# torognes/vsearch

Measured on AMD Instinct MI355X. Metric: GCUPS (useful DP cells/s of the search16 global-alignment path: DP + traceback + CIGAR), higher is better.
Workload: dtype int16

## Files before the change

### vsearch_amd/csrc/vsx_device.hip

```cpp
#include <hip/hip_runtime.h>
#include <type_traits>
#include <cstdlib>
#include <atomic>
#include "vsx_internal.h"

typedef unsigned int u32;
typedef unsigned int u32x4 __attribute__((ext_vector_type(4)));
typedef unsigned int u32x3 __attribute__((ext_vector_type(3)));
typedef short s2 __attribute__((ext_vector_type(2)));
typedef unsigned short us2 __attribute__((ext_vector_type(2)));

#define DEV __device__ __forceinline__
struct __attribute__((aligned(4))) Pair2 { unsigned int x, y; };

#define SIGN2 0x80008000u

DEV s2 S2(u32 x) { return __builtin_bit_cast(s2, x); }
DEV us2 U2(u32 x) { return __builtin_bit_cast(us2, x); }
DEV u32 UI(s2 x) { return __builtin_bit_cast(u32, x); }
DEV u32 UI(us2 x) { return __builtin_bit_cast(u32, x); }

DEV u32 sadd(u32 a, u32 b) { return UI(__builtin_elementwise_add_sat(S2(a), S2(b))); }
DEV u32 ssub(u32 a, u32 b) { return UI(__builtin_elementwise_sub_sat(S2(a), S2(b))); }
DEV u32 pmax(u32 a, u32 b) { return UI(__builtin_elementwise_max(S2(a), S2(b))); }
// ... 814 lines not shown
  static DEV u32 max(u32 a, u32 b) { return (u32) __builtin_elementwise_max((unsigned short) a, (unsigned short) b); }
  static DEV u32 dif(u32 a, u32 b) { return a - b; }
  static DEV u32 neg(u32 d) { return d >> 31; }
  static DEV u32 fun(u32 acc, u32 d) { return __builtin_amdgcn_alignbit(acc, d, 31); }
  static DEV u32 one_row_word(u32 acc) { return acc << 12; }
  static DEV u32 nibble(u32 w, int rows_in_group, int y) { return (w >> (4 * (rows_in_group - 1 - y))) & 15u; }
  static constexpr u32 UP = 8, LEFT = 4, EXT_UP = 2, EXT_LEFT = 1;
};

typedef u32 u32_unaligned __attribute__((aligned(1)));
typedef unsigned long long u64_unaligned __attribute__((aligned(1)));
struct __attribute__((aligned(4))) Quad { u32 x, y, z, w; };
struct __attribute__((aligned(4))) Trio { u32 x, y, z; };

#include "vsx_accept.h"

#ifndef VSX_TB_STATS
#define VSX_TB_STATS 0
#endif
#if VSX_TB_STATS
__device__ unsigned long long vsx_tb_stats_dev[16];
extern "C" hipError_t vsx_internal_tb_stats(unsigned long long * out8, int reset)
{
  hipError_t e = hipMemcpyFromSymbol(out8, HIP_SYMBOL(vsx_tb_stats_dev), sizeof(unsigned long long) * 16);
  if (e == hipSuccess && reset) { unsigned long long z[16] = {0}; e = hipMemcpyToSymbol(HIP_SYMBOL(vsx_tb_stats_dev), z, sizeof z); }
  return e;
}
#endif

#ifndef VSX_TB_WAVES
#define VSX_TB_WAVES(R_, MID_) ((MID_) ? ((R_) <= 24 ? 4 : 3) : ((R_) <= 12 ? 4 : ((R_) <= 16 ? 3 : 2)))
#endif
template <int R, bool FAST, bool CK8 = false, bool MID = false>
__global__ void __launch_bounds__(128) __attribute__((amdgpu_waves_per_eu(VSX_TB_WAVES(R, MID), 8)))
vsx_traceback_ck_kernel(const VsxDevParams P, const VsxFilterDev FL, const VsxTask * __restrict__ tasks,
                        const u32 * __restrict__ pair_slot, const u32 * __restrict__ pair_ids, u32 npairs,
                        const uint8_t * __restrict__ qc, const uint8_t * __restrict__ tc,
                        const u32 * __restrict__ ck, const VsxSlotOut * __restrict__ slot,
                        u32 * __restrict__ slab, const uint64_t * __restrict__ slab_off,
                        u32 * __restrict__ runs, uint64_t runs_capacity, unsigned long long * cursor,
                        VsxPairOut * __restrict__ out)
{
  typedef TbOps<FAST> A;
  static_assert(VSX_RB == 1, "the tile staging below reads row checkpoints as two-step (16-byte) pairs");
  static_assert(!CK8 || FAST, "compressed checkpoints belong to the TILT class");
  static_assert(!MID || (CK8 && R % 2 == 0), "half-height tiles belong to the TILT class");
  constexpr int RT = MID ? R / 2 : R;
  constexpr int ND = (RT + 3) / 4;
  constexpr bool TOPPAD = FAST;
  typedef typename std::conditional<CK8, uint8_t, int16_t>::type SshT;
  __shared__ SshT Ssh[512];
  __shared__ uint16_t bitsL_all[2 * 16 * ND * 64];
  __shared__ u32 tbL_all[2 * 17 * 64];
  __shared__ uint8_t symL_all[2 * 8 * 64];
  const int tid = (int) (threadIdx.x & 63);
  const int wv = (int) (threadIdx.x >> 6);
// ... 375 lines not shown
              if (op == 1 && (bts & A::EXT_LEFT)) { --j; push(1); }
              else if (op == 2 && (bts & A::EXT_UP)) { --i; --r; push(2); }
              else if (bts & A::LEFT) { if (op != 1) ++ga; --j; push(1); }
              else if (bts & A::UP) { if (op != 2) ++ga; --i; --r; push(2); }
              else { --i; --r; --j; push(0); }
#if VSX_TB_STATS
              atomicAdd(&vsx_tb_stats_dev[3], 1ull);
#endif
            }
          if (r < 0 && L > 0) { --L; r = (L == 0 ? rtop0 : R) - 1; }
        }
    }
#if VSX_TB_STATS
  if (valid) atomicAdd(&vsx_tb_stats_dev[5], 1ull);
#endif
  if (!valid) return;

  VsxPairOut o;
  o.pad = 0; o.nruns = 0; o.run_off = 0;
  if (so.overflow)
    {
      o.score = 32767; o.aligned = 0; o.matches = 0; o.mismatches = 0; o.gaps = 0;
      out[pair_ids[k]] = o;
      rank_note(FL, pair_ids[k], 0u, 32767, 0.0);
      return;
    }
  if (i >= 0) { al += (u32) (i + 1); if (op != 2) ++ga; push_n(2, (u32) (i + 1)); }
  if (j >= 0) { al += (u32) (j + 1); if (op != 1) ++ga; push_n(1, (u32) (j + 1)); }
  if (op >= 0) my[nruns++] = (runlen << 2) | (u32) op;

  u32 ma = 0, mi = 0;
  {
    int qi = Q - 1, tj = D - 1;
    for (u32 x = 0; x < nruns; ++x)
      {
        const u32 w = my[x];
        const int len = (int) (w >> 2);
        const u32 o2 = w & 3u;
        if (o2 == 0)
          {
            for (int b = 0; b < len; b += 8)
              {
                const int rem = (len - b < 8) ? len - b : 8;
                const unsigned long long aw = *reinterpret_cast<const u64_unaligned *>(q + (qi - b - 7));
                const unsigned long long cw = *reinterpret_cast<const u64_unaligned *>(d + (tj - b - 7));
                const unsigned long long ones = 0x0101010101010101ull;
                const unsigned long long x = aw & cw;
                unsigned long long t = (x | (x >> 1) | (x >> 2) | (x >> 3)) & ones;
                if (P.n_mismatch)
                  {
                    const unsigned long long a15 = aw & (aw >> 1) & (aw >> 2) & (aw >> 3);
                    const unsigned long long c15 = cw & (cw >> 1) & (cw >> 2) & (cw >> 3);
                    t &= ~(a15 | c15);
                  }
                t &= ~0ull << (8 * (8 - rem));
                const u32 m8 = (u32) __builtin_popcountll(t);
                ma += m8;
                mi += (u32) rem - m8;
              }
            qi -= len; tj -= len;
          }
        else if (o2 == 1) tj -= len;
        else qi -= len;
      }
  }

  u32 verdict = 0;
  double idv = 0.0;
  if (FL.enabled && nruns > 0) verdict = accept_verdict(FL, Q, D, (int) al, (int) ma, (int) mi, (int) ga, my[nruns - 1], my[0], &idv);
  if (verdict == 3u) nruns = 0;
  rank_note(FL, pair_ids[k], verdict, (int) so.score, idv);

  const unsigned long long base = atomicAdd(cursor, (unsigned long long) nruns);
  if (base + nruns <= runs_capacity)
    for (u32 x = 0; x < nruns; ++x) runs[base + x] = my[x];

  o.score = so.score;
  o.aligned = (uint16_t) al; o.matches = (uint16_t) ma; o.mismatches = (uint16_t) mi; o.gaps = (uint16_t) ga;
  o.pad = (uint16_t) verdict;
  o.nruns = nruns;
  o.run_off = base;
  out[pair_ids[k]] = o;
}


DEV u32 pk_add(u32 a, u32 b) { return UI((us2) (U2(a) + U2(b))); }
DEV u32 pk_sub(u32 a, u32 b) { return psubw(a, b); }
#ifdef VSX_TB2_WAVES_N
#define VSX_TB2_WAVES(R_, MID_) VSX_TB2_WAVES_N
#endif
#ifndef VSX_TB2_WAVES
#define VSX_TB2_WAVES(R_, MID_) 3
#endif
#ifndef VSX_TB_LDSSTAGE
#define VSX_TB_LDSSTAGE 1
#endif
#ifndef VSX_TB_LDSSTAGE_FOR
#define VSX_TB_LDSSTAGE_FOR(R_) ((R_) == 14 || (R_) == 16 || (R_) >= 26)
#endif
#ifndef VSX_TB_WALK_BATCH
#define VSX_TB_WALK_BATCH 4
#endif
static_assert(VSX_TB_WALK_BATCH >= 1 && VSX_TB_WALK_BATCH <= 16, "a batch stays inside one 16-column tile");
template <int R, bool MID>
__global__ void __launch_bounds__(64) __attribute__((amdgpu_waves_per_eu(VSX_TB2_WAVES(R, MID), 8)))
vsx_traceback_tilt_kernel(const VsxDevParams P, const VsxFilterDev FL, const VsxTask * __restrict__ tasks,
                          const u32 * __restrict__ pair_slot, const u32 * __restrict__ pair_ids, u32 npairs,
                          const uint8_t * __restrict__ qc, const uint8_t * __restrict__ tc,
                          const u32 * __restrict__ ck, const VsxSlotOut * __restrict__ slot,
                          u32 * __restrict__ slab, const uint64_t * __restrict__ slab_off,
                          u32 * __restrict__ runs, uint64_t runs_capacity, unsigned long long * cursor,
                          VsxPairOut * __restrict__ out)
{
  static_assert(R >= 4 && (!MID || R % 2 == 0), "R = 1 keeps the first kernel");
  constexpr int RT = MID ? R / 2 : R;
  constexpr int HR = (RT + 1) / 2;
  constexpr int NG = (HR + 3) / 4;
  constexpr int XL = RT - 1 - HR;
  constexpr int WB = VSX_TB_WALK_BATCH;
  constexpr int NBQ = MID ? VSX_COLCK_NBH(RT) : VSX_COLCK_NB(R, true);
  __shared__ uint8_t Ssh[512];
  __shared__ u32 Ssh4[16];
  constexpr int BITS_DW = 17 * NG * 64, SYM_DW = 10 * 64 / 4;
  __shared__ __attribute__((aligned(16))) u32 arenaL[BITS_DW + SYM_DW + 19 * 64];
  u32 * const bitsL = arenaL;
  uint8_t * const symL = reinterpret_cast<uint8_t *>(arenaL + BITS_DW);
  u32 * const tbL = arenaL + BITS_DW + SYM_DW;
// ... 458 lines not shown
#endif
          TBMARK(3 * tno + 2);
        }
      if (busy && r < 0 && L > 0) { --L; r = R - 1; }
    }
#if VSX_TB_STATS
  if (valid) atomicAdd(&vsx_tb_stats_dev[5], 1ull);
  if (n_cells) atomicAdd(&vsx_tb_stats_dev[3], (unsigned long long) n_cells);
  if (tid == 0)
    {
      atomicAdd(&vsx_tb_stats_dev[15], __builtin_readcyclecounter() - t_kernel0); atomicAdd(&vsx_tb_stats_dev[0], (unsigned long long) n_iter);
      atomicAdd(&vsx_tb_stats_dev[4], (unsigned long long) n_trips);
      for (int k2 = 0; k2 < 6; ++k2) atomicAdd(&vsx_tb_stats_dev[8 + k2], tphase[k2]);
    }
#endif
  if (!valid) return;

  VsxPairOut o;
  o.pad = 0; o.nruns = 0; o.run_off = 0;
  if (so.overflow)
    {
      o.score = 32767; o.aligned = 0; o.matches = 0; o.mismatches = 0; o.gaps = 0;
      out[pair_ids[k]] = o;
      rank_note(FL, pair_ids[k], 0u, 32767, 0.0);
      return;
    }
  if (i >= 0) { al += (u32) (i + 1); if (op != 2) ++ga; push_n(2, (u32) (i + 1)); }
  if (j >= 0) { al += (u32) (j + 1); if (op != 1) ++ga; push_n(1, (u32) (j + 1)); }
  if (op >= 0) my[nruns++] = (runlen << 2) | (u32) op;

  u32 ma = 0, mi = 0;
  {
    int qi = Q - 1, tj = D - 1;
    for (u32 x = 0; x < nruns; ++x)
      {
        const u32 w = my[x];
        const int len = (int) (w >> 2);
        const u32 o2 = w & 3u;
        if (o2 == 0)
          {
            for (int b = 0; b < len; b += 8)
              {
                const int rem = (len - b < 8) ? len - b : 8;
                const unsigned long long aw = *reinterpret_cast<const u64_unaligned *>(q + (qi - b - 7));
                const unsigned long long cw = *reinterpret_cast<const u64_unaligned *>(d + (tj - b - 7));
                const unsigned long long ones = 0x0101010101010101ull;
                const unsigned long long x2 = aw & cw;
                unsigned long long t = (x2 | (x2 >> 1) | (x2 >> 2) | (x2 >> 3)) & ones;
                if (P.n_mismatch)
                  {
                    const unsigned long long a15 = aw & (aw >> 1) & (aw >> 2) & (aw >> 3);
                    const unsigned long long c15 = cw & (cw >> 1) & (cw >> 2) & (cw >> 3);
                    t &= ~(a15 | c15);
                  }
                t &= ~0ull << (8 * (8 - rem));
                const u32 m8 = (u32) __builtin_popcountll(t);
                ma += m8;
                mi += (u32) rem - m8;
              }
            qi -= len; tj -= len;
          }
        else if (o2 == 1) tj -= len;
        else qi -= len;
      }
  }

  u32 verdict = 0;
  double idv = 0.0;
  if (FL.enabled && nruns > 0) verdict = accept_verdict(FL, Q, D, (int) al, (int) ma, (int) mi, (int) ga, my[nruns - 1], my[0], &idv);
  if (verdict == 3u) nruns = 0;
  rank_note(FL, pair_ids[k], verdict, (int) so.score, idv);

  const unsigned long long base = atomicAdd(cursor, (unsigned long long) nruns);
  if (base + nruns <= runs_capacity)
    for (u32 x = 0; x < nruns; ++x) runs[base + x] = my[x];

  o.score = so.score;
  o.aligned = (uint16_t) al; o.matches = (uint16_t) ma; o.mismatches = (uint16_t) mi; o.gaps = (uint16_t) ga;
  o.pad = (uint16_t) verdict;
  o.nruns = nruns;
  o.run_off = base;
  out[pair_ids[k]] = o;
}

DEV u32 map4(u32 ch)
{
  const u32 c = ch | 0x20u;
  if (((ch | 0x20u) < 'a') || ((ch | 0x20u) > 'z') || ((ch & 0xC0u) != 0x40u)) return 0;
  switch (c)
    {
    case 'a': return 1;  case 'b': return 14; case 'c': return 2;  case 'd': return 13;
    case 'g': return 4;  case 'h': return 11; case 'k': return 12; case 'm': return 3;
    case 'n': return 15; case 'r': return 5;  case 's': return 6;  case 't': return 8;
    case 'u': return 8;  case 'v': return 7;  case 'w': return 9;  case 'y': return 10;
    default: return 0;
    }
}
// ... 169 lines not shown
{
  if (ntasks == 0) return hipSuccess;
#define FWDR(RR) case RR: return launch_fwd2<RR>(track, nq, one, P, d_tasks, ntasks, q, t, dir, strip, slot, st)
  switch (rows)
    {
    FWDR(1); FWDR(4); FWDR(8); FWDR(10); FWDR(12); FWDR(14); FWDR(16); FWDR(18); FWDR(20); FWDR(22); FWDR(24); FWDR(26); FWDR(28); FWDR(32);
    default: return hipErrorInvalidValue;
    }
#undef FWDR
}

template <int R, bool MID>
static hipError_t launch_tbtilt(const VsxDevParams & P, const VsxFilterDev & F, const VsxTask * d_tasks, const uint32_t * d_pair_slot,
                                const uint32_t * d_pair_ids, uint32_t npairs, const uint8_t * q, const uint8_t * t,
                                const uint32_t * ck, const VsxSlotOut * slot, uint32_t * slab, const uint64_t * slab_off,
                                uint32_t * runs, uint64_t cap, unsigned long long * cursor, VsxPairOut * out, hipStream_t st)
{
  if constexpr (R >= 4)
    hipLaunchKernelGGL((vsx_traceback_tilt_kernel<R, MID>), dim3((npairs + 63) / 64), dim3(64), 0, st,
                       P, F, d_tasks, d_pair_slot, d_pair_ids, npairs, q, t, ck, slot, slab, slab_off, runs, cap, cursor, out);
  return hipGetLastError();
}

template <int R, bool FAST, bool CK8 = false, bool MID = false>
static hipError_t launch_tbck(const VsxDevParams & P, const VsxFilterDev & F, const VsxTask * d_tasks, const uint32_t * d_pair_slot,
                              const uint32_t * d_pair_ids, uint32_t npairs, const uint8_t * q, const uint8_t * t,
                              const uint32_t * ck, const VsxSlotOut * slot, uint32_t * slab, const uint64_t * slab_off,
                              uint32_t * runs, uint64_t cap, unsigned long long * cursor, VsxPairOut * out, hipStream_t st)
{
  hipLaunchKernelGGL((vsx_traceback_ck_kernel<R, FAST, CK8, MID>), dim3((npairs + 127) / 128), dim3(128), 0, st,
                     P, F, d_tasks, d_pair_slot, d_pair_ids, npairs, q, t, ck, slot, slab, slab_off, runs, cap, cursor, out);
  return hipGetLastError();
}

extern "C" hipError_t vsx_launch_traceback_ck(int rows, int fast16, VsxDevParams P, VsxFilterDev F, const VsxTask * d_tasks, const uint32_t * d_pair_slot,
                                              const uint32_t * d_pair_ids, uint32_t npairs,
                                              const uint8_t * q, const uint8_t * t,
                                              const uint32_t * ck, const VsxSlotOut * slot,
                                              uint32_t * slab, const uint64_t * slab_off,
                                              uint32_t * runs, uint64_t runs_capacity, unsigned long long * cursor,
                                              VsxPairOut * out, hipStream_t st)
{
  if (npairs == 0) return hipSuccess;
  int dev_now = 0;
  if (hipGetDevice(&dev_now) != hipSuccess) { (void) hipGetLastError(); dev_now = 64; }
  const bool v2 = g_tb_v1_dev[dev_now < 0 || dev_now > 64 ? 64 : dev_now].load(std::memory_order_relaxed) == 0;
#define TBCK(RR) case RR: return (fast16 && P.tilt != 0 && v2 && RR >= 4) ? launch_tbtilt<RR, VSX_MID(RR, true)>(P, F, d_tasks, d_pair_slot, d_pair_ids, npairs, q, t, ck, slot, slab, slab_off, runs, runs_capacity, cursor, out, st) \
                                 : (fast16 && P.tilt != 0) ? launch_tbck<RR, true, true, VSX_MID(RR, true)>(P, F, d_tasks, d_pair_slot, d_pair_ids, npairs, q, t, ck, slot, slab, slab_off, runs, runs_capacity, cursor, out, st) \
                                 : fast16 ? launch_tbck<RR, true>(P, F, d_tasks, d_pair_slot, d_pair_ids, npairs, q, t, ck, slot, slab, slab_off, runs, runs_capacity, cursor, out, st) \
                                        : launch_tbck<RR, false>(P, F, d_tasks, d_pair_slot, d_pair_ids, npairs, q, t, ck, slot, slab, slab_off, runs, runs_capacity, cursor, out, st)
  switch (rows)
    {
    TBCK(1); TBCK(4); TBCK(8); TBCK(10); TBCK(12); TBCK(14); TBCK(16); TBCK(18); TBCK(20); TBCK(22); TBCK(24); TBCK(26); TBCK(28); TBCK(32);
    default: return hipErrorInvalidValue;
    }
#undef TBCK
}

extern "C" uint64_t vsx_ckpt_dwords(uint64_t nstrips, uint64_t steps, uint64_t rows, int tilt)
{
  const uint64_t nblk = (steps + 15) >> 4;
  const uint64_t rowck = (((nstrips * steps) + 1) >> 1) * VSX_ROWCK_PAIR_DW(tilt != 0);
  if (tilt)
    {
      const bool mid = VSX_MID(rows, true);
// ... 8 lines not shown
```

### vsearch_amd/csrc/vsx_host.cpp

```cpp
#include "../../include/vsx.h"
#include "vsx_internal.h"
#include "vsx_private.h"

#include <hip/hip_runtime.h>
#include <algorithm>
#include <cerrno>
#include <cinttypes>
#include <cstdio>
#include <cstdlib>
#include <cstring>
#include <sched.h>
#include <thread>
#include <atomic>
#include <condition_variable>
#include <mutex>
#include <chrono>
#include <deque>
#include <functional>
#include <memory>
#include <numeric>
#include <string>
#include <vector>

using vsxp::fail;
// ... 1456 lines not shown
  pl->filter.refused_pair = pl->d_refused_pair.p;
  return VSX_OK;
}

int vsx_plan_run(vsx_plan * pl)
{
  if (!pl) return fail(VSX_EINVAL, "vsx_plan_run: null plan");
  vsx_ctx * ctx = pl->ctx;
  VSX_HIP(hipSetDevice(ctx->device));
  hipStream_t st = pl->alt_fwd ? ctx->stream_b : ctx->stream, st2 = ctx->stream2;
  const int slot = pl->dir_slot;
  const int poison = vsx_internal_poison_byte();
  VSX_HIP(hipMemsetAsync(pl->d_cursor.p, 0, 3 * sizeof(unsigned long long), st));
  if (pl->filter.rank_counts) VSX_HIP(hipMemsetAsync(pl->d_rank_counts.p, 0, 2 * sizeof(uint32_t), st));
  VSX_HIP(hipEventRecord(pl->ev_begin, st));
  for (size_t k = 0; k < pl->chunks.size(); ++k)
    {
      Chunk & c = pl->chunks[k];
      uint32_t * dir = pl->d_dir[0].p;
      if (k >= 1) VSX_HIP(hipStreamWaitEvent(st, pl->chunks[k - 1].e2, 0));
      else if (ctx->ev_tb_used[slot]) VSX_HIP(hipStreamWaitEvent(st, ctx->ev_tb[slot], 0));
      if (poison >= 0)
        {
          VSX_HIP(hipMemsetAsync(dir, poison, (c.dir_dwords + VSX_CK_SLACK_DW) * sizeof(uint32_t), st));
          if (c.strip_elems) VSX_HIP(hipMemsetAsync(pl->d_strip.p, poison, c.strip_elems * sizeof(uint2), st));
        }
      VSX_HIP(hipEventRecord(c.e0, st));
      for (const Launch & L : c.launches)
        {
          VsxDevParams Pf = L.tilt ? ctx->Pt : ctx->P;
// ... 8 lines not shown
      VSX_HIP(hipStreamWaitEvent(st2, c.e1, 0));
      if (poison >= 0 && c.slab_words) VSX_HIP(hipMemsetAsync(pl->d_slab.p, poison, c.slab_words * sizeof(uint32_t), st2));
      VSX_HIP(hipEventRecord(c.e1b, st2));
      for (size_t li = 0; li < c.launches.size();)
        {
          const Launch & L = c.launches[li];
          uint32_t pair_count = L.pair_count;
          size_t lj = li + 1;
          while (lj < c.launches.size() && c.launches[lj].rows == L.rows &&
                 c.launches[lj].track == L.track && c.launches[lj].tilt == L.tilt) { pair_count += c.launches[lj].pair_count; ++lj; }
          VsxDevParams Pb = L.tilt ? ctx->Pt : ctx->P;
          Pb.max3 = (L.tilt == 2) ? 1 : 0;
          VSX_HIP(vsx_launch_traceback_ck(L.rows, L.track == 0 ? 1 : 0, Pb, pl->filter, pl->d_tasks.p, pl->d_pair_slot.p + L.pair_first,
                                         pl->d_pair_ids.p + L.pair_first, pair_count, pl->Q->codes(), pl->T->codes(),
                                         dir, pl->d_slot.p, pl->d_slab.p, pl->d_slab_off.p + L.pair_first,
                                         pl->d_runs.p, pl->runs_capacity, pl->d_cursor.p, pl->d_out.p, st2));
          li = lj;
        }
      VSX_HIP(hipEventRecord(c.e2, st2));
    }
  if (pl->chunks.empty()) VSX_HIP(hipStreamWaitEvent(st2, pl->ev_begin, 0));
  VSX_HIP(hipEventRecord(ctx->ev_tb[slot], st2));
  ctx->ev_tb_used[slot] = true;
  VSX_HIP(vsx_launch_cigar_text(pl->d_out.p, pl->d_pair_ids.p, (uint32_t) pl->pair_ids.size(), pl->d_runs.p, pl->runs_capacity,
                               pl->d_text.p, pl->text_capacity, pl->d_cursor.p + 1, pl->soa, st2));
  VSX_HIP(hipMemcpyAsync(pl->h_cursor, pl->d_cursor.p, 3 * sizeof(unsigned long long), hipMemcpyDeviceToHost, st2));
  VSX_HIP(hipEventRecord(pl->ev_end, st2));
  pl->ran = true;
  pl->host_patched = false;
  return VSX_OK;
}

int vsx_plan_sync(vsx_plan * pl, vsx_timing * tm)
{
  if (!pl) return fail(VSX_EINVAL, "vsx_plan_sync: null plan");
  if (!pl->ran) return fail(VSX_EINVAL, "vsx_plan_sync: plan has not been run");
  VSX_HIP(hipSetDevice(pl->ctx->device));
  VSX_HIP(hipEventSynchronize(pl->ev_end));
  if (tm)
    {
// ... 622 lines not shown
```

### vsearch_amd/csrc/vsx_internal.h

```cpp
#ifndef VSX_INTERNAL_H
#define VSX_INTERNAL_H

#include <stdint.h>
#include <hip/hip_runtime_api.h>

#define VSX_TASK_SLOTS 8
#define VSX_GROUP_LANES 16
#define VSX_MAX_SEQLEN_SUM 65535LL
#define VSX_MAX_SEQLEN_PRODUCT 25000000LL
#define VSX_TABLE_LEN (65536 + 64)
#define VSX_CODE_SLACK 64
#define VSX_CK_SLACK_DW 4096
#ifndef VSX_MID_MIN_ROWS
#define VSX_MID_MIN_ROWS 18
#endif
#define VSX_MID(R_, TILT_) ((TILT_) && (R_) >= VSX_MID_MIN_ROWS)
#define VSX_SPLIT_ROWS(R_) ((R_) == 10 || (R_) == 16)

struct VsxDevParams {
  uint32_t match_pk;
  uint32_t qrq_i_pk, rq_i_pk;
  uint32_t qrq_r_pk, rq_r_pk;
  int32_t  qrt_i, rt_i;
  int32_t  qrt_r, rt_r;
  int32_t  match, mismatch;
  int32_t  smin;
  int32_t  n_mismatch;
  int32_t  share_sub;
  int32_t  top_open, top_step;
  int32_t  tilt;
  int32_t  max3;
  int32_t  es_on, es_w0, es_e, es_rr, es_rate;
// ... 35 lines not shown
struct VsxPairOut {
  int16_t  score;
  uint16_t aligned, matches, mismatches, gaps;
  uint16_t pad;
  uint32_t nruns;
  uint64_t run_off;
};

struct VsxSoaOut {
  int16_t  * score;
  uint16_t * aligned, * matches, * mismatches, * gaps;
  uint8_t  * verdict;
  uint64_t * text_off;
};

struct VsxRankedOut {
  uint32_t * pair;
  int16_t  * score;
  uint16_t * aligned, * matches, * mismatches, * gaps;
  uint8_t  * verdict;
  double   * id;
  uint64_t * text_off;
};

#define VSX_CHIM_MAXCAND 16
struct VsxChimItem {
  uint32_t q;
  uint32_t ncand;
  uint32_t pair0;
  uint32_t out;
// ... 47 lines not shown
hipError_t vsx_launch_revcomp(uint8_t * d_codes, const uint64_t * d_src_off, const uint64_t * d_dst_off,
                              const uint32_t * d_len, uint64_t nseq, hipStream_t st);

hipError_t vsx_launch_encode(const uint8_t * d_ascii, uint8_t * d_codes, uint64_t nbytes, hipStream_t st);
hipError_t vsx_launch_purity(const uint8_t * d_codes, const uint64_t * d_off, const uint32_t * d_len,
                             uint64_t nseq, uint8_t * d_impure, hipStream_t st);
hipError_t vsx_launch_forward(int rows, int track, int nq, int one , VsxDevParams P, const VsxTask * d_tasks, uint32_t ntasks,
                              const uint8_t * d_qcodes, const uint8_t * d_tcodes,
                              uint32_t * d_dir, uint2 * d_strip, VsxSlotOut * d_slot, hipStream_t st);
hipError_t vsx_launch_traceback_ck(int rows, int fast16, VsxDevParams P, VsxFilterDev F, const VsxTask * d_tasks, const uint32_t * d_pair_slot,
                                   const uint32_t * d_pair_ids, uint32_t npairs,
                                   const uint8_t * d_qcodes, const uint8_t * d_tcodes,
                                   const uint32_t * d_ck, const VsxSlotOut * d_slot,
                                   uint32_t * d_slab, const uint64_t * d_slab_off,
                                   uint32_t * d_runs, uint64_t runs_capacity, unsigned long long * d_cursor,
                                   VsxPairOut * d_out, hipStream_t st);
hipError_t vsx_launch_max3_selftest(uint32_t * d_bad , hipStream_t st);
void vsx_internal_set_tb_v2(int device, int on);
uint64_t vsx_ckpt_dwords(uint64_t nstrips, uint64_t steps, uint64_t rows, int tilt );
const int * vsx_supported_rows(int * count);

hipError_t vsx_kmer_launch_sweep(int fill, const uint8_t * codes, const uint64_t * off, const uint32_t * len,
                                 const uint32_t * seq_list, uint32_t nseq, int w, uint32_t ntiles, uint32_t * bucket_count,
                                 const uint64_t * bucket_start, uint32_t * postings, const uint8_t * lower_bits, hipStream_t st);
hipError_t vsx_kmer_launch_case_bits(const uint8_t * d_ascii, uint64_t nbytes, uint8_t * d_bits , int fold_case,
                                     hipStream_t st);
hipError_t vsx_launch_dust(const uint8_t * d_codes, const uint64_t * d_off, const uint32_t * d_len, uint64_t nseq, uint8_t * d_bits,
                           hipStream_t st);
hipError_t vsx_kmer_launch_ranges(const uint64_t * bucket_start, uint32_t ntiles, const uint64_t * qk_start, const uint32_t * qk,
                                  const uint32_t * minmatch, const uint32_t * qlist, uint32_t nslots, void * ranges, hipStream_t st);
hipError_t vsx_kmer_launch_count(int bits, int tagged, const uint32_t * postings, const uint64_t * bucket_start, const void * ranges,
// ... 25 lines not shown
```

### vsearch_amd/csrc/vsx_tbtext.hip

```cpp
#include <hip/hip_runtime.h>
#include "vsx_internal.h"

typedef unsigned int u32;

#define DEV __device__ __forceinline__

DEV u32 ndigits(u32 v) { return v >= 10000u ? 5u : v >= 1000u ? 4u : v >= 100u ? 3u : v >= 10u ? 2u : 1u; }

__global__ void __launch_bounds__(256)
vsx_cigar_text_kernel(const VsxPairOut * __restrict__ out, const u32 * __restrict__ pair_ids, u32 npairs,
                      const u32 * __restrict__ runs, uint64_t runs_capacity,
                      uint8_t * __restrict__ text, uint64_t text_capacity, unsigned long long * text_cursor,
                      VsxSoaOut soa)
{
  const u32 k = blockIdx.x * blockDim.x + threadIdx.x;
  const bool valid = k < npairs;
  const u32 pid = valid ? pair_ids[k] : 0u;
  VsxPairOut o {};
  if (valid) o = out[pid];
  const bool have_runs = valid && (o.run_off + o.nruns <= runs_capacity);
  const u32 * __restrict__ my = runs + o.run_off;
  const u32 nruns = have_runs ? o.nruns : 0u;

  u32 len = 1;
  for (u32 x = 0; x < nruns; ++x)
    {
      const u32 n = my[x] >> 2;
      len += 1u + (n > 1u ? ndigits(n) : 0u);
    }
  const u32 len4 = valid ? ((len + 3u) & ~3u) : 0u;

  u32 incl = len4;
#pragma unroll
  for (int d = 1; d < 64; d <<= 1)
    {
      const u32 v = (u32) __shfl_up((int) incl, d, 64);
      if ((int) (threadIdx.x & 63) >= d) incl += v;
    }
  const u32 total = (u32) __shfl((int) incl, 63, 64);
  unsigned long long base = 0;
  if ((threadIdx.x & 63) == 0 && total) base = atomicAdd(text_cursor, (unsigned long long) total);
  base = (unsigned long long) __shfl((long long) base, 0, 64);
  if (!valid) return;
  const unsigned long long off = base + (unsigned long long) (incl - len4);

  if (off + len4 <= text_capacity)
    {
      u32 * __restrict__ dst = reinterpret_cast<u32 *>(text + off);
      u32 acc = 0, have = 0;
      auto put = [&](u32 ch) {
        acc |= ch << (8u * have);
        if (++have == 4u) { *dst++ = acc; acc = 0; have = 0; }
      };
      for (u32 x = nruns; x-- > 0;)
        {
          const u32 w = my[x];
          const u32 n = w >> 2;
          if (n > 1u)
            {
              if (n >= 10000u) put('0' + n / 10000u);
              if (n >= 1000u) put('0' + (n / 1000u) % 10u);
              if (n >= 100u) put('0' + (n / 100u) % 10u);
              if (n >= 10u) put('0' + (n / 10u) % 10u);
              put('0' + n % 10u);
            }
          put((w & 3u) == 0u ? 'M' : (w & 3u) == 1u ? 'I' : 'D');
        }
      put(0u);
      if (have) *dst = acc;
    }

  soa.score[pid] = o.score;
  soa.aligned[pid] = o.aligned;
  soa.matches[pid] = o.matches;
  soa.mismatches[pid] = o.mismatches;
  soa.gaps[pid] = o.gaps;
  soa.verdict[pid] = (uint8_t) o.pad;
  soa.text_off[pid] = off;
}

__global__ void __launch_bounds__(256)
vsx_revcomp_kernel(const uint8_t * __restrict__ codes, const uint64_t * __restrict__ src_off, const uint64_t * __restrict__ dst_off,
                   const uint32_t * __restrict__ len)
{
  const uint64_t k = blockIdx.x;
  const uint8_t * __restrict__ s = codes + src_off[k];
  uint8_t * __restrict__ d = const_cast<uint8_t *>(codes) + dst_off[k];
  const u32 L = len[k];
  for (u32 x = threadIdx.x; x < L; x += 256)
    {
      const u32 c = s[L - 1 - x] & 15u;
      const u32 r = ((c & 1u) << 3) | ((c & 2u) << 1) | ((c & 4u) >> 1) | ((c & 8u) >> 3);
      d[x] = (uint8_t) (c == 0u ? 15u : r);
// ... 22 lines not shown
```

Measured before the change: 9578.

## Fuse CIGAR text formatting into traceback kernels

The traceback kernels now format the CIGAR text and write the SoA outputs themselves, using a wave-wide prefix scan to allocate text space. This replaces the separate cigar-text kernel launch, so the run words no longer go to global memory and come back. The writer fills the string back to front so runs can be emitted in stored order. The trade is extra registers and work in the traceback kernels, and the early returns are restructured so every lane reaches the wave-wide shuffle.

```diff
diff --git a/vsearch_amd/csrc/vsx_device.hip b/vsearch_amd/csrc/vsx_device.hip
--- a/vsearch_amd/csrc/vsx_device.hip
+++ b/vsearch_amd/csrc/vsx_device.hip
@@ -852,6 +852,7 @@
 struct __attribute__((aligned(4))) Trio { u32 x, y, z; };
 
 #include "vsx_accept.h"
+#include "vsx_tbtext.h"
 
 #ifndef VSX_TB_STATS
 #define VSX_TB_STATS 0
@@ -877,7 +878,7 @@
                         const u32 * __restrict__ ck, const VsxSlotOut * __restrict__ slot,
                         u32 * __restrict__ slab, const uint64_t * __restrict__ slab_off,
                         u32 * __restrict__ runs, uint64_t runs_capacity, unsigned long long * cursor,
-                        VsxPairOut * __restrict__ out)
+                        VsxPairOut * __restrict__ out, const VsxTextOut TX)
 {
   typedef TbOps<FAST> A;
   static_assert(VSX_RB == 1, "the tile staging below reads row checkpoints as two-step (16-byte) pairs");
@@ -1283,73 +1284,83 @@
 #if VSX_TB_STATS
   if (valid) atomicAdd(&vsx_tb_stats_dev[5], 1ull);
 #endif
-  if (!valid) return;
-
+  const u32 pid = valid ? pair_ids[k] : 0u;
+  bool have_runs = true;
+  u32 tlen = 1;
   VsxPairOut o;
   o.pad = 0; o.nruns = 0; o.run_off = 0;
-  if (so.overflow)
-    {
-      o.score = 32767; o.aligned = 0; o.matches = 0; o.mismatches = 0; o.gaps = 0;
-      out[pair_ids[k]] = o;
-      rank_note(FL, pair_ids[k], 0u, 32767, 0.0);
-      return;
-    }
-  if (i >= 0) { al += (u32) (i + 1); if (op != 2) ++ga; push_n(2, (u32) (i + 1)); }
-  if (j >= 0) { al += (u32) (j + 1); if (op != 1) ++ga; push_n(1, (u32) (j + 1)); }
-  if (op >= 0) my[nruns++] = (runlen << 2) | (u32) op;
-
-  u32 ma = 0, mi = 0;
-  {
-    int qi = Q - 1, tj = D - 1;
-    for (u32 x = 0; x < nruns; ++x)
+  o.score = 32767; o.aligned = 0; o.matches = 0; o.mismatches = 0; o.gaps = 0;
+  if (valid && so.overflow)
+    {
+      out[pid] = o;
+      rank_note(FL, pid, 0u, 32767, 0.0);
+    }
+  if (live)
+    {
+      if (i >= 0) { al += (u32) (i + 1); if (op != 2) ++ga; push_n(2, (u32) (i + 1)); }
+      if (j >= 0) { al += (u32) (j + 1); if (op != 1) ++ga; push_n(1, (u32) (j + 1)); }
+      if (op >= 0) my[nruns++] = (runlen << 2) | (u32) op;
+
+      u32 ma = 0, mi = 0;
       {
-        const u32 w = my[x];
-        const int len = (int) (w >> 2);
-        const u32 o2 = w & 3u;
-        if (o2 == 0)
+        int qi = Q - 1, tj = D - 1;
+        for (u32 x = 0; x < nruns; ++x)
           {
-            for (int b = 0; b < len; b += 8)
+            const u32 w = my[x];
+            const int len = (int) (w >> 2);
+            if (VSX_TB_FUSED_TEXT) tlen += vsx_cigar_run_len(w);
+            const u32 o2 = w & 3u;
+            if (o2 == 0)
               {
-                const int rem = (len - b < 8) ? len - b : 8;
-                const unsigned long long aw = *reinterpret_cast<const u64_unaligned *>(q + (qi - b - 7));
-                const unsigned long long cw = *reinterpret_cast<const u64_unaligned *>(d + (tj - b - 7));
-                const unsigned long long ones = 0x0101010101010101ull;
-                const unsigned long long x = aw & cw;
-                unsigned long long t = (x | (x >> 1) | (x >> 2) | (x >> 3)) & ones;
-                if (P.n_mismatch)
+                for (int b = 0; b < len; b += 8)
                   {
-                    const unsigned long long a15 = aw & (aw >> 1) & (aw >> 2) & (aw >> 3);
-                    const unsigned long long c15 = cw & (cw >> 1) & (cw >> 2) & (cw >> 3);
-                    t &= ~(a15 | c15);
+                    const int rem = (len - b < 8) ? len - b : 8;
+                    const unsigned long long aw = *reinterpret_cast<const u64_unaligned *>(q + (qi - b - 7));
+                    const unsigned long long cw = *reinterpret_cast<const u64_unaligned *>(d + (tj - b - 7));
+                    const unsigned long long ones = 0x0101010101010101ull;
+                    const unsigned long long x = aw & cw;
+                    unsigned long long t = (x | (x >> 1) | (x >> 2) | (x >> 3)) & ones;
+                    if (P.n_mismatch)
+                      {
+                        const unsigned long long a15 = aw & (aw >> 1) & (aw >> 2) & (aw >> 3);
+                        const unsigned long long c15 = cw & (cw >> 1) & (cw >> 2) & (cw >> 3);
+                        t &= ~(a15 | c15);
+                      }
+                    t &= ~0ull << (8 * (8 - rem));
+                    const u32 m8 = (u32) __builtin_popcountll(t);
+                    ma += m8;
+                    mi += (u32) rem - m8;
                   }
-                t &= ~0ull << (8 * (8 - rem));
-                const u32 m8 = (u32) __builtin_popcountll(t);
-                ma += m8;
-                mi += (u32) rem - m8;
+                qi -= len; tj -= len;
               }
-            qi -= len; tj -= len;
+            else if (o2 == 1) tj -= len;
+            else qi -= len;
           }
-        else if (o2 == 1) tj -= len;
-        else qi -= len;
       }
-  }
-
-  u32 verdict = 0;
-  double idv = 0.0;
-  if (FL.enabled && nruns > 0) verdict = accept_verdict(FL, Q, D, (int) al, (int) ma, (int) mi, (int) ga, my[nruns - 1], my[0], &idv);
-  if (verdict == 3u) nruns = 0;
-  rank_note(FL, pair_ids[k], verdict, (int) so.score, idv);
-
-  const unsigned long long base = atomicAdd(cursor, (unsigned long long) nruns);
-  if (base + nruns <= runs_capacity)
-    for (u32 x = 0; x < nruns; ++x) runs[base + x] = my[x];
-
-  o.score = so.score;
-  o.aligned = (uint16_t) al; o.matches = (uint16_t) ma; o.mismatches = (uint16_t) mi; o.gaps = (uint16_t) ga;
-  o.pad = (uint16_t) verdict;
-  o.nruns = nruns;
-  o.run_off = base;
-  out[pair_ids[k]] = o;
+
+      u32 verdict = 0;
+      double idv = 0.0;
+      if (FL.enabled && nruns > 0) verdict = accept_verdict(FL, Q, D, (int) al, (int) ma, (int) mi, (int) ga, my[nruns - 1], my[0], &idv);
+      if (verdict == 3u) nruns = 0;
+      rank_note(FL, pid, verdict, (int) so.score, idv);
+
+      const unsigned long long base = atomicAdd(cursor, (unsigned long long) nruns);
+      have_runs = base + nruns <= runs_capacity;
+      if (!VSX_TB_FUSED_TEXT && have_runs)
+        for (u32 x = 0; x < nruns; ++x) runs[base + x] = my[x];
+
+      o.score = so.score;
+      o.aligned = (uint16_t) al; o.matches = (uint16_t) ma; o.mismatches = (uint16_t) mi; o.gaps = (uint16_t) ga;
+      o.pad = (uint16_t) verdict;
+      o.nruns = nruns;
+      o.run_off = base;
+      out[pid] = o;
+    }
+#if VSX_TB_FUSED_TEXT
+  vsx_marshal_pair(valid, pid, o, my, have_runs ? o.nruns : 0u, tlen, runs, TX);
+#else
+  (void) tlen;
+#endif
 }
 
 
@@ -1379,7 +1390,7 @@
                           const u32 * __restrict__ ck, const VsxSlotOut * __restrict__ slot,
                           u32 * __restrict__ slab, const uint64_t * __restrict__ slab_off,
                           u32 * __restrict__ runs, uint64_t runs_capacity, unsigned long long * cursor,
-                          VsxPairOut * __restrict__ out)
+                          VsxPairOut * __restrict__ out, const VsxTextOut TX)
 {
   static_assert(R >= 4 && (!MID || R % 2 == 0), "R = 1 keeps the first kernel");
   constexpr int RT = MID ? R / 2 : R;
@@ -1868,73 +1879,83 @@
       for (int k2 = 0; k2 < 6; ++k2) atomicAdd(&vsx_tb_stats_dev[8 + k2], tphase[k2]);
     }
 #endif
-  if (!valid) return;
-
+  const u32 pid = valid ? pair_ids[k] : 0u;
+  bool have_runs = true;
+  u32 tlen = 1;
   VsxPairOut o;
   o.pad = 0; o.nruns = 0; o.run_off = 0;
-  if (so.overflow)
-    {
-      o.score = 32767; o.aligned = 0; o.matches = 0; o.mismatches = 0; o.gaps = 0;
-      out[pair_ids[k]] = o;
-      rank_note(FL, pair_ids[k], 0u, 32767, 0.0);
-      return;
-    }
-  if (i >= 0) { al += (u32) (i + 1); if (op != 2) ++ga; push_n(2, (u32) (i + 1)); }
-  if (j >= 0) { al += (u32) (j + 1); if (op != 1) ++ga; push_n(1, (u32) (j + 1)); }
-  if (op >= 0) my[nruns++] = (runlen << 2) | (u32) op;
-
-  u32 ma = 0, mi = 0;
-  {
-    int qi = Q - 1, tj = D - 1;
-    for (u32 x = 0; x < nruns; ++x)
+  o.score = 32767; o.aligned = 0; o.matches = 0; o.mismatches = 0; o.gaps = 0;
+  if (valid && so.overflow)
+    {
+      out[pid] = o;
+      rank_note(FL, pid, 0u, 32767, 0.0);
+    }
+  if (live)
+    {
+      if (i >= 0) { al += (u32) (i + 1); if (op != 2) ++ga; push_n(2, (u32) (i + 1)); }
+      if (j >= 0) { al += (u32) (j + 1); if (op != 1) ++ga; push_n(1, (u32) (j + 1)); }
+      if (op >= 0) my[nruns++] = (runlen << 2) | (u32) op;
+
+      u32 ma = 0, mi = 0;
       {
-        const u32 w = my[x];
-        const int len = (int) (w >> 2);
-        const u32 o2 = w & 3u;
-        if (o2 == 0)
+        int qi = Q - 1, tj = D - 1;
+        for (u32 x = 0; x < nruns; ++x)
           {
-            for (int b = 0; b < len; b += 8)
+            const u32 w = my[x];
+            const int len = (int) (w >> 2);
+            if (VSX_TB_FUSED_TEXT) tlen += vsx_cigar_run_len(w);
+            const u32 o2 = w & 3u;
+            if (o2 == 0)
               {
-                const int rem = (len - b < 8) ? len - b : 8;
-                const unsigned long long aw = *reinterpret_cast<const u64_unaligned *>(q + (qi - b - 7));
-                const unsigned long long cw = *reinterpret_cast<const u64_unaligned *>(d + (tj - b - 7));
-                const unsigned long long ones = 0x0101010101010101ull;
-                const unsigned long long x2 = aw & cw;
-                unsigned long long t = (x2 | (x2 >> 1) | (x2 >> 2) | (x2 >> 3)) & ones;
-                if (P.n_mismatch)
+                for (int b = 0; b < len; b += 8)
                   {
-                    const unsigned long long a15 = aw & (aw >> 1) & (aw >> 2) & (aw >> 3);
-                    const unsigned long long c15 = cw & (cw >> 1) & (cw >> 2) & (cw >> 3);
-                    t &= ~(a15 | c15);
+                    const int rem = (len - b < 8) ? len - b : 8;
+                    const unsigned long long aw = *reinterpret_cast<const u64_unaligned *>(q + (qi - b - 7));
+                    const unsigned long long cw = *reinterpret_cast<const u64_unaligned *>(d + (tj - b - 7));
+                    const unsigned long long ones = 0x0101010101010101ull;
+                    const unsigned long long x2 = aw & cw;
+                    unsigned long long t = (x2 | (x2 >> 1) | (x2 >> 2) | (x2 >> 3)) & ones;
+                    if (P.n_mismatch)
+                      {
+                        const unsigned long long a15 = aw & (aw >> 1) & (aw >> 2) & (aw >> 3);
+                        const unsigned long long c15 = cw & (cw >> 1) & (cw >> 2) & (cw >> 3);
+                        t &= ~(a15 | c15);
+                      }
+                    t &= ~0ull << (8 * (8 - rem));
+                    const u32 m8 = (u32) __builtin_popcountll(t);
+                    ma += m8;
+                    mi += (u32) rem - m8;
                   }
-                t &= ~0ull << (8 * (8 - rem));
-                const u32 m8 = (u32) __builtin_popcountll(t);
-                ma += m8;
-                mi += (u32) rem - m8;
+                qi -= len; tj -= len;
               }
-            qi -= len; tj -= len;
+            else if (o2 == 1) tj -= len;
+            else qi -= len;
           }
-        else if (o2 == 1) tj -= len;
-        else qi -= len;
       }
-  }
-
-  u32 verdict = 0;
-  double idv = 0.0;
-  if (FL.enabled && nruns > 0) verdict = accept_verdict(FL, Q, D, (int) al, (int) ma, (int) mi, (int) ga, my[nruns - 1], my[0], &idv);
-  if (verdict == 3u) nruns = 0;
-  rank_note(FL, pair_ids[k], verdict, (int) so.score, idv);
-
-  const unsigned long long base = atomicAdd(cursor, (unsigned long long) nruns);
-  if (base + nruns <= runs_capacity)
-    for (u32 x = 0; x < nruns; ++x) runs[base + x] = my[x];
-
-  o.score = so.score;
-  o.aligned = (uint16_t) al; o.matches = (uint16_t) ma; o.mismatches = (uint16_t) mi; o.gaps = (uint16_t) ga;
-  o.pad = (uint16_t) verdict;
-  o.nruns = nruns;
-  o.run_off = base;
-  out[pair_ids[k]] = o;
+
+      u32 verdict = 0;
+      double idv = 0.0;
+      if (FL.enabled && nruns > 0) verdict = accept_verdict(FL, Q, D, (int) al, (int) ma, (int) mi, (int) ga, my[nruns - 1], my[0], &idv);
+      if (verdict == 3u) nruns = 0;
+      rank_note(FL, pid, verdict, (int) so.score, idv);
+
+      const unsigned long long base = atomicAdd(cursor, (unsigned long long) nruns);
+      have_runs = base + nruns <= runs_capacity;
+      if (!VSX_TB_FUSED_TEXT && have_runs)
+        for (u32 x = 0; x < nruns; ++x) runs[base + x] = my[x];
+
+      o.score = so.score;
+      o.aligned = (uint16_t) al; o.matches = (uint16_t) ma; o.mismatches = (uint16_t) mi; o.gaps = (uint16_t) ga;
+      o.pad = (uint16_t) verdict;
+      o.nruns = nruns;
+      o.run_off = base;
+      out[pid] = o;
+    }
+#if VSX_TB_FUSED_TEXT
+  vsx_marshal_pair(valid, pid, o, my, have_runs ? o.nruns : 0u, tlen, runs, TX);
+#else
+  (void) tlen;
+#endif
 }
 
 DEV u32 map4(u32 ch)
@@ -2134,11 +2155,11 @@
 static hipError_t launch_tbtilt(const VsxDevParams & P, const VsxFilterDev & F, const VsxTask * d_tasks, const uint32_t * d_pair_slot,
                                 const uint32_t * d_pair_ids, uint32_t npairs, const uint8_t * q, const uint8_t * t,
                                 const uint32_t * ck, const VsxSlotOut * slot, uint32_t * slab, const uint64_t * slab_off,
-                                uint32_t * runs, uint64_t cap, unsigned long long * cursor, VsxPairOut * out, hipStream_t st)
+                                uint32_t * runs, uint64_t cap, unsigned long long * cursor, VsxPairOut * out, const VsxTextOut & tx, hipStream_t st)
 {
   if constexpr (R >= 4)
     hipLaunchKernelGGL((vsx_traceback_tilt_kernel<R, MID>), dim3((npairs + 63) / 64), dim3(64), 0, st,
-                       P, F, d_tasks, d_pair_slot, d_pair_ids, npairs, q, t, ck, slot, slab, slab_off, runs, cap, cursor, out);
+                       P, F, d_tasks, d_pair_slot, d_pair_ids, npairs, q, t, ck, slot, slab, slab_off, runs, cap, cursor, out, tx);
   return hipGetLastError();
 }
 
@@ -2146,10 +2167,10 @@
 static hipError_t launch_tbck(const VsxDevParams & P, const VsxFilterDev & F, const VsxTask * d_tasks, const uint32_t * d_pair_slot,
                               const uint32_t * d_pair_ids, uint32_t npairs, const uint8_t * q, const uint8_t * t,
                               const uint32_t * ck, const VsxSlotOut * slot, uint32_t * slab, const uint64_t * slab_off,
-                              uint32_t * runs, uint64_t cap, unsigned long long * cursor, VsxPairOut * out, hipStream_t st)
+                              uint32_t * runs, uint64_t cap, unsigned long long * cursor, VsxPairOut * out, const VsxTextOut & tx, hipStream_t st)
 {
   hipLaunchKernelGGL((vsx_traceback_ck_kernel<R, FAST, CK8, MID>), dim3((npairs + 127) / 128), dim3(128), 0, st,
-                     P, F, d_tasks, d_pair_slot, d_pair_ids, npairs, q, t, ck, slot, slab, slab_off, runs, cap, cursor, out);
+                     P, F, d_tasks, d_pair_slot, d_pair_ids, npairs, q, t, ck, slot, slab, slab_off, runs, cap, cursor, out, tx);
   return hipGetLastError();
 }
 
@@ -2159,16 +2180,16 @@
                                               const uint32_t * ck, const VsxSlotOut * slot,
                                               uint32_t * slab, const uint64_t * slab_off,
                                               uint32_t * runs, uint64_t runs_capacity, unsigned long long * cursor,
-                                              VsxPairOut * out, hipStream_t st)
+                                              VsxPairOut * out, VsxTextOut tx, hipStream_t st)
 {
   if (npairs == 0) return hipSuccess;
   int dev_now = 0;
   if (hipGetDevice(&dev_now) != hipSuccess) { (void) hipGetLastError(); dev_now = 64; }
   const bool v2 = g_tb_v1_dev[dev_now < 0 || dev_now > 64 ? 64 : dev_now].load(std::memory_order_relaxed) == 0;
-#define TBCK(RR) case RR: return (fast16 && P.tilt != 0 && v2 && RR >= 4) ? launch_tbtilt<RR, VSX_MID(RR, true)>(P, F, d_tasks, d_pair_slot, d_pair_ids, npairs, q, t, ck, slot, slab, slab_off, runs, runs_capacity, cursor, out, st) \
-                                 : (fast16 && P.tilt != 0) ? launch_tbck<RR, true, true, VSX_MID(RR, true)>(P, F, d_tasks, d_pair_slot, d_pair_ids, npairs, q, t, ck, slot, slab, slab_off, runs, runs_capacity, cursor, out, st) \
-                                 : fast16 ? launch_tbck<RR, true>(P, F, d_tasks, d_pair_slot, d_pair_ids, npairs, q, t, ck, slot, slab, slab_off, runs, runs_capacity, cursor, out, st) \
-                                        : launch_tbck<RR, false>(P, F, d_tasks, d_pair_slot, d_pair_ids, npairs, q, t, ck, slot, slab, slab_off, runs, runs_capacity, cursor, out, st)
+#define TBCK(RR) case RR: return (fast16 && P.tilt != 0 && v2 && RR >= 4) ? launch_tbtilt<RR, VSX_MID(RR, true)>(P, F, d_tasks, d_pair_slot, d_pair_ids, npairs, q, t, ck, slot, slab, slab_off, runs, runs_capacity, cursor, out, tx, st) \
+                                 : (fast16 && P.tilt != 0) ? launch_tbck<RR, true, true, VSX_MID(RR, true)>(P, F, d_tasks, d_pair_slot, d_pair_ids, npairs, q, t, ck, slot, slab, slab_off, runs, runs_capacity, cursor, out, tx, st) \
+                                 : fast16 ? launch_tbck<RR, true>(P, F, d_tasks, d_pair_slot, d_pair_ids, npairs, q, t, ck, slot, slab, slab_off, runs, runs_capacity, cursor, out, tx, st) \
+                                        : launch_tbck<RR, false>(P, F, d_tasks, d_pair_slot, d_pair_ids, npairs, q, t, ck, slot, slab, slab_off, runs, runs_capacity, cursor, out, tx, st)
   switch (rows)
     {
     TBCK(1); TBCK(4); TBCK(8); TBCK(10); TBCK(12); TBCK(14); TBCK(16); TBCK(18); TBCK(20); TBCK(22); TBCK(24); TBCK(26); TBCK(28); TBCK(32);
diff --git a/vsearch_amd/csrc/vsx_host.cpp b/vsearch_amd/csrc/vsx_host.cpp
--- a/vsearch_amd/csrc/vsx_host.cpp
+++ b/vsearch_amd/csrc/vsx_host.cpp
@@ -1494,6 +1494,7 @@
   VSX_HIP(hipMemsetAsync(pl->d_cursor.p, 0, 3 * sizeof(unsigned long long), st));
   if (pl->filter.rank_counts) VSX_HIP(hipMemsetAsync(pl->d_rank_counts.p, 0, 2 * sizeof(uint32_t), st));
   VSX_HIP(hipEventRecord(pl->ev_begin, st));
+  const VsxTextOut tx {pl->d_text.p, pl->text_capacity, pl->d_cursor.p + 1, pl->soa};
   for (size_t k = 0; k < pl->chunks.size(); ++k)
     {
       Chunk & c = pl->chunks[k];
@@ -1532,7 +1533,7 @@
           VSX_HIP(vsx_launch_traceback_ck(L.rows, L.track == 0 ? 1 : 0, Pb, pl->filter, pl->d_tasks.p, pl->d_pair_slot.p + L.pair_first,
                                          pl->d_pair_ids.p + L.pair_first, pair_count, pl->Q->codes(), pl->T->codes(),
                                          dir, pl->d_slot.p, pl->d_slab.p, pl->d_slab_off.p + L.pair_first,
-                                         pl->d_runs.p, pl->runs_capacity, pl->d_cursor.p, pl->d_out.p, st2));
+                                         pl->d_runs.p, pl->runs_capacity, pl->d_cursor.p, pl->d_out.p, tx, st2));
           li = lj;
         }
       VSX_HIP(hipEventRecord(c.e2, st2));
@@ -1540,8 +1541,9 @@
   if (pl->chunks.empty()) VSX_HIP(hipStreamWaitEvent(st2, pl->ev_begin, 0));
   VSX_HIP(hipEventRecord(ctx->ev_tb[slot], st2));
   ctx->ev_tb_used[slot] = true;
-  VSX_HIP(vsx_launch_cigar_text(pl->d_out.p, pl->d_pair_ids.p, (uint32_t) pl->pair_ids.size(), pl->d_runs.p, pl->runs_capacity,
-                               pl->d_text.p, pl->text_capacity, pl->d_cursor.p + 1, pl->soa, st2));
+  if (!VSX_TB_FUSED_TEXT || pl->chunks.empty())
+    VSX_HIP(vsx_launch_cigar_text(pl->d_out.p, pl->d_pair_ids.p, (uint32_t) pl->pair_ids.size(), pl->d_runs.p, pl->runs_capacity,
+                                 pl->d_text.p, pl->text_capacity, pl->d_cursor.p + 1, pl->soa, st2));
   VSX_HIP(hipMemcpyAsync(pl->h_cursor, pl->d_cursor.p, 3 * sizeof(unsigned long long), hipMemcpyDeviceToHost, st2));
   VSX_HIP(hipEventRecord(pl->ev_end, st2));
   pl->ran = true;
diff --git a/vsearch_amd/csrc/vsx_internal.h b/vsearch_amd/csrc/vsx_internal.h
--- a/vsearch_amd/csrc/vsx_internal.h
+++ b/vsearch_amd/csrc/vsx_internal.h
@@ -16,6 +16,9 @@
 #endif
 #define VSX_MID(R_, TILT_) ((TILT_) && (R_) >= VSX_MID_MIN_ROWS)
 #define VSX_SPLIT_ROWS(R_) ((R_) == 10 || (R_) == 16)
+#ifndef VSX_TB_FUSED_TEXT
+#define VSX_TB_FUSED_TEXT 1
+#endif
 
 struct VsxDevParams {
   uint32_t match_pk;
@@ -81,6 +84,13 @@
   uint64_t * text_off;
 };
 
+struct VsxTextOut {
+  uint8_t * text;
+  uint64_t text_capacity;
+  unsigned long long * text_cursor;
+  VsxSoaOut soa;
+};
+
 struct VsxRankedOut {
   uint32_t * pair;
   int16_t  * score;
@@ -158,7 +168,7 @@
                                    const uint32_t * d_ck, const VsxSlotOut * d_slot,
                                    uint32_t * d_slab, const uint64_t * d_slab_off,
                                    uint32_t * d_runs, uint64_t runs_capacity, unsigned long long * d_cursor,
-                                   VsxPairOut * d_out, hipStream_t st);
+                                   VsxPairOut * d_out, VsxTextOut tx, hipStream_t st);
 hipError_t vsx_launch_max3_selftest(uint32_t * d_bad , hipStream_t st);
 void vsx_internal_set_tb_v2(int device, int on);
 uint64_t vsx_ckpt_dwords(uint64_t nstrips, uint64_t steps, uint64_t rows, int tilt );
diff --git a/vsearch_amd/csrc/vsx_tbtext.h b/vsearch_amd/csrc/vsx_tbtext.h
--- /dev/null
+++ b/vsearch_amd/csrc/vsx_tbtext.h
@@ -0,0 +1,102 @@
+#ifndef VSX_TBTEXT_H
+#define VSX_TBTEXT_H
+
+#include <hip/hip_runtime.h>
+#include "vsx_internal.h"
+
+__host__ __device__ inline uint32_t vsx_cigar_ndigits(uint32_t v)
+{
+  return v >= 10000u ? 5u : v >= 1000u ? 4u : v >= 100u ? 3u : v >= 10u ? 2u : 1u;
+}
+
+__host__ __device__ inline uint32_t vsx_cigar_run_len(uint32_t w)
+{
+  const uint32_t n = w >> 2;
+  return 1u + (n > 1u ? vsx_cigar_ndigits(n) : 0u);
+}
+
+__host__ __device__ inline uint32_t vsx_cigar_len(const uint32_t * runs, uint32_t nruns)
+{
+  uint32_t len = 1;
+  for (uint32_t x = 0; x < nruns; ++x) len += vsx_cigar_run_len(runs[x]);
+  return len;
+}
+
+struct VsxCigarWriter {
+  uint32_t * dst;
+  uint32_t acc;
+  int p;
+  __host__ __device__ VsxCigarWriter(uint32_t * d, uint32_t len) : dst(d), acc(0), p((int) len - 1) {}
+  __host__ __device__ void put(uint32_t ch)
+  {
+    acc |= ch << (8u * ((uint32_t) p & 3u));
+    if ((p & 3) == 0) { dst[p >> 2] = acc; acc = 0; }
+    --p;
+  }
+  __host__ __device__ void begin() { put(0u); }
+  __host__ __device__ void run(uint32_t w)
+  {
+    uint32_t n = w >> 2;
+    put((w & 3u) == 0u ? 'M' : (w & 3u) == 1u ? 'I' : 'D');
+    if (n > 1u)
+      do { put('0' + n % 10u); n /= 10u; } while (n);
+  }
+};
+
+__host__ __device__ inline void vsx_cigar_format(const uint32_t * runs, uint32_t nruns, uint32_t * dst)
+{
+  VsxCigarWriter W(dst, vsx_cigar_len(runs, nruns));
+  W.begin();
+  for (uint32_t x = 0; x < nruns; ++x) W.run(runs[x]);
+}
+
+#ifdef __HIPCC__
+__device__ inline unsigned long long vsx_text_alloc(uint32_t len4, unsigned long long * text_cursor)
+{
+  const uint32_t lane = (uint32_t) threadIdx.x & 63u;
+  uint32_t incl = len4;
+#pragma unroll
+  for (int d = 1; d < 64; d <<= 1)
+    {
+      const uint32_t v = (uint32_t) __shfl_up((int) incl, d, 64);
+      if ((int) lane >= d) incl += v;
+    }
+  const uint32_t total = (uint32_t) __shfl((int) incl, 63, 64);
+  unsigned long long base = 0;
+  if (lane == 0 && total) base = atomicAdd(text_cursor, (unsigned long long) total);
+  base = (unsigned long long) __shfl((long long) base, 0, 64);
+  return base + (unsigned long long) (incl - len4);
+}
+
+__device__ inline void vsx_soa_store(const VsxSoaOut & soa, uint32_t pid, const VsxPairOut & o, unsigned long long text_off)
+{
+  soa.score[pid] = o.score;
+  soa.aligned[pid] = o.aligned;
+  soa.matches[pid] = o.matches;
+  soa.mismatches[pid] = o.mismatches;
+  soa.gaps[pid] = o.gaps;
+  soa.verdict[pid] = (uint8_t) o.pad;
+  soa.text_off[pid] = text_off;
+}
+
+__device__ inline void vsx_marshal_pair(bool valid, uint32_t pid, const VsxPairOut & o, const uint32_t * my, uint32_t nw, uint32_t text_len,
+                                        uint32_t * runs, const VsxTextOut & tx)
+{
+  if (nw == 0) text_len = 1;
+  const uint32_t len4 = valid ? ((text_len + 3u) & ~3u) : 0u;
+  const unsigned long long off = vsx_text_alloc(len4, tx.text_cursor);
+  if (!valid) return;
+  const bool fits = off + len4 <= tx.text_capacity;
+  VsxCigarWriter W(reinterpret_cast<uint32_t *>(tx.text + off), text_len);
+  if (fits) W.begin();
+  for (uint32_t x = 0; x < nw; ++x)
+    {
+      const uint32_t w = my[x];
+      runs[o.run_off + x] = w;
+      if (fits) W.run(w);
+    }
+  vsx_soa_store(tx.soa, pid, o, off);
+}
+#endif
+
+#endif
diff --git a/vsearch_amd/csrc/vsx_tbtext.hip b/vsearch_amd/csrc/vsx_tbtext.hip
--- a/vsearch_amd/csrc/vsx_tbtext.hip
+++ b/vsearch_amd/csrc/vsx_tbtext.hip
@@ -1,11 +1,8 @@
 #include <hip/hip_runtime.h>
 #include "vsx_internal.h"
+#include "vsx_tbtext.h"
 
 typedef unsigned int u32;
-
-#define DEV __device__ __forceinline__
-
-DEV u32 ndigits(u32 v) { return v >= 10000u ? 5u : v >= 1000u ? 4u : v >= 100u ? 3u : v >= 10u ? 2u : 1u; }
 
 __global__ void __launch_bounds__(256)
 vsx_cigar_text_kernel(const VsxPairOut * __restrict__ out, const u32 * __restrict__ pair_ids, u32 npairs,
@@ -21,62 +18,18 @@
   const bool have_runs = valid && (o.run_off + o.nruns <= runs_capacity);
   const u32 * __restrict__ my = runs + o.run_off;
   const u32 nruns = have_runs ? o.nruns : 0u;
+  const u32 len4 = valid ? ((vsx_cigar_len(my, nruns) + 3u) & ~3u) : 0u;
+  const unsigned long long off = vsx_text_alloc(len4, text_cursor);
+  if (!valid) return;
+  if (off + len4 <= text_capacity) vsx_cigar_format(my, nruns, reinterpret_cast<u32 *>(text + off));
+  vsx_soa_store(soa, pid, o, off);
+}
 
-  u32 len = 1;
-  for (u32 x = 0; x < nruns; ++x)
-    {
-      const u32 n = my[x] >> 2;
-      len += 1u + (n > 1u ? ndigits(n) : 0u);
-    }
-  const u32 len4 = valid ? ((len + 3u) & ~3u) : 0u;
-
-  u32 incl = len4;
-#pragma unroll
-  for (int d = 1; d < 64; d <<= 1)
-    {
-      const u32 v = (u32) __shfl_up((int) incl, d, 64);
-      if ((int) (threadIdx.x & 63) >= d) incl += v;
-    }
-  const u32 total = (u32) __shfl((int) incl, 63, 64);
-  unsigned long long base = 0;
-  if ((threadIdx.x & 63) == 0 && total) base = atomicAdd(text_cursor, (unsigned long long) total);
-  base = (unsigned long long) __shfl((long long) base, 0, 64);
-  if (!valid) return;
-  const unsigned long long off = base + (unsigned long long) (incl - len4);
-
-  if (off + len4 <= text_capacity)
-    {
-      u32 * __restrict__ dst = reinterpret_cast<u32 *>(text + off);
-      u32 acc = 0, have = 0;
-      auto put = [&](u32 ch) {
-        acc |= ch << (8u * have);
-        if (++have == 4u) { *dst++ = acc; acc = 0; have = 0; }
-      };
-      for (u32 x = nruns; x-- > 0;)
-        {
-          const u32 w = my[x];
-          const u32 n = w >> 2;
-          if (n > 1u)
-            {
-              if (n >= 10000u) put('0' + n / 10000u);
-              if (n >= 1000u) put('0' + (n / 1000u) % 10u);
-              if (n >= 100u) put('0' + (n / 100u) % 10u);
-              if (n >= 10u) put('0' + (n / 10u) % 10u);
-              put('0' + n % 10u);
-            }
-          put((w & 3u) == 0u ? 'M' : (w & 3u) == 1u ? 'I' : 'D');
-        }
-      put(0u);
-      if (have) *dst = acc;
-    }
-
-  soa.score[pid] = o.score;
-  soa.aligned[pid] = o.aligned;
-  soa.matches[pid] = o.matches;
-  soa.mismatches[pid] = o.mismatches;
-  soa.gaps[pid] = o.gaps;
-  soa.verdict[pid] = (uint8_t) o.pad;
-  soa.text_off[pid] = off;
+extern "C" uint32_t vsx_internal_cigar_format(const uint32_t * runs, uint32_t nruns, uint8_t * dst, uint32_t dst_bytes)
+{
+  const uint32_t len4 = (vsx_cigar_len(runs, nruns) + 3u) & ~3u;
+  if (len4 <= dst_bytes) vsx_cigar_format(runs, nruns, reinterpret_cast<uint32_t *>(dst));
+  return len4;
 }
 
 __global__ void __launch_bounds__(256)
```

Result: faster. 9676 (median of 6 runs) (+1.0%).
